# yumcyaWiz/fredholm

Hardware: AMD Instinct MI355X
Metric: Msamples/s at 1920x1080, max_depth=8 (higher is better)
Workload: dtype f32; 1 GPU; configs[2]: 1M random-triangle soup (PCG32 seed 0x853c49e6748fea9b), Hosek sky turbidity 3 albedo 0.3, 1920x1080, max_depth 8, seed 1; triangles=1000000, parallelism=single GPU, gather=none, post=none

## Files before the change

### fredholm_amd/csrc/capi.hip

```cpp
#include <hip/hip_runtime.h>

#include <cmath>
#include <cstdlib>
#include <cstring>

#include "../../include/fredholm/image_io.h"
#include <hip/hip_gl_interop.h>

#include "context.h"
#include "fh_bsdf.h"
#include "fh_local_exposure.h"
#include "fh_meter.h"
#include "fh_trace.h"

#include "gen/tables.inc"

namespace fh {

static thread_local std::string g_create_error;

int fail(fh_ctx* ctx, int code, const std::string& msg)
{
  g_create_error = msg;
  if (ctx) ctx->err = msg;
// ... 154 lines not shown
    int v = 0;
    if (hipDeviceGetAttribute(&v, hipDeviceAttributeMaxSharedMemoryPerMultiprocessor, device) == hipSuccess && v >= 64 * 1024) t.lds_per_cu = (uint32_t)v;
    if (hipDeviceGetAttribute(&v, hipDeviceAttributeSharedMemPerBlockOptin, device) == hipSuccess && v >= 64 * 1024) t.lds_per_block = (uint32_t)v;
    if (t.lds_per_block > t.lds_per_cu) t.lds_per_block = t.lds_per_cu;
    auto env_uint = [](const char* name, int lo, int hi, uint32_t& dst) { if (const char* e = getenv(name)) { const int v = atoi(e); if (v >= lo && v <= hi) dst = (uint32_t)v; } };
    auto env_off = [](const char* name, bool& dst) { if (const char* e = getenv(name)) dst = e[0] != '0'; };
    env_uint("FH_COOP_T", 1, 64, t.coop_flush);
    t.coop_flush_fixed = getenv("FH_COOP_T") != nullptr;
    env_off("FH_COOP", t.coop);
    env_off("FH_STREAM", t.stream);
    t.stream_forced = t.stream && getenv("FH_STREAM") != nullptr;
    env_uint("FH_STREAM_REFILL", 1, 64, t.stream_refill);
    env_uint("FH_STREAM_MIN_RAYS", 0, 65535, t.stream_min_rays);
    env_off("FH_SORT_SMALL", t.sort_small);
    env_off("FH_OVERLAP", t.overlap_secondary);
    env_off("FH_MERGE", t.merge_trace);
    env_uint("FH_SKY_BLOCKS", 0, 64, t.sky_blocks_per_cu);
    env_uint("FH_SKY_FILLER_GRID", 0, 65535, t.sky_filler_grid);
    if (const char* e = getenv("FH_POISON")) t.poison_pools = e[0] == '1';
    env_off("FH_SKY_SPLIT", t.sky_split);
    env_uint("FH_SKY_SPLIT_MIN_LOG2", 0, 40, t.sky_split_min_log2);
    env_uint("FH_STACK_LDS", 1, 99, t.stack_lds_entries);
    env_uint("FH_SHADE_WGS", 2, 3, t.shade_wgs);
    env_uint("FH_STREAM_CHUNK", 16, 65535, t.stream_chunk);
    t.stream_chunk_fixed = getenv("FH_STREAM_CHUNK") != nullptr;
    if (t.stream_chunk_fixed) t.stream_chunk_closest = t.stream_chunk;
    env_uint("FH_STREAM_CHUNK_CLOSEST", 16, 65535, t.stream_chunk_closest);
    env_uint("FH_TAIL_DEPTH", 0, 64, t.tail_depth);
    env_uint("FH_TAIL_PATHS", 64, 1 << 30, t.tail_paths);
    env_off("FH_SORT", t.sort_queues);
    env_uint("FH_SORT_ONEPASS", 0, 2, t.sort_onepass);
    env_uint("FH_BOTTOM_UP", 0, 2, t.bottom_up);
    env_uint("FH_SKY_DEFER", 0, 1, t.sky_defer);
    t.debug_tail = getenv("FH_DEBUG_TAIL") != nullptr;
    if (const char* e = getenv("FH_FORCE_ALPHA")) t.force_alpha = e[0] == '1';
  }
  {
    int least = 0, greatest = 0;
    const char* e = getenv("FH_SKY_PRIO");
    const bool low = !(e && e[0] == '0') && hipDeviceGetStreamPriorityRange(&least, &greatest) == hipSuccess;
    if (ctx->sky_stream.create(hipStreamNonBlocking, low ? least : 0) != hipSuccess) return bail("stream creation failed");
  }
  if (ctx->ev_sky.create(hipEventDisableTiming) != hipSuccess || ctx->ev_sky_cursor.create(hipEventDisableTiming) != hipSuccess) return bail("event creation failed");
  if (ctx->d_split_counters.alloc(4) != hipSuccess) return bail("device allocation failed");
  (void)hipMemsetAsync(ctx->d_split_counters, 0, 16, ctx->stream);
  if (ctx->ev_render_begin.create() != hipSuccess || ctx->ev_render_end.create() != hipSuccess) return bail("event creation failed");
  if (hipStreamSynchronize(ctx->stream) != hipSuccess) return bail("hipStreamSynchronize failed");
  *out = ctx;
  return FH_OK;
}

int fh_ctx_destroy(fh_ctx* ctx)
{
  FH_GROUP(ctx, group_destroy(ctx));
  if (!ctx) return FH_E_INVALID;
  (void)hipSetDevice(ctx->device);
  (void)drain_passes(ctx, true);
  delete ctx;
  return FH_OK;
}

const char* fh_last_error(fh_ctx* ctx) { return ctx ? ctx->err.c_str() : g_create_error.c_str(); }

int fh_set_flags(fh_ctx* ctx, uint32_t flags)
{
  FH_GROUP_EACH(ctx, kGroupCallPlain, fh_set_flags(m_, flags));
  CTX_CHECK(ctx);
  ctx->flags = flags;
  return FH_OK;
}
int fh_get_flags(fh_ctx* ctx, uint32_t* flags)
{
  FH_GROUP_LEAD(ctx);
  CTX_CHECK(ctx);
  if (!flags) return fail(ctx, FH_E_INVALID, "fh_get_flags: null argument");
  *flags = ctx->flags;
  return FH_OK;
}
// ... 783 lines not shown
```

### fredholm_amd/csrc/context.h

```cpp
#pragma once
#include <hip/hip_runtime.h>

#include <functional>
#include <string>
#include <vector>

#include "../../include/fredholm_hip.h"
#include "fh_device.h"
#include "fh_envmap.h"
#include "fh_lights.h"
#include "fh_memory.h"
#include "temporal_host.h"

struct fh_group;

namespace fh { constexpr int kPassSlots = 3; }

struct fh_ctx {
  fh_group* group = nullptr;
  fh_ctx* owner = nullptr;
  uint32_t member_index = 0;
  int device = 0;
  fh::Stream stream;
  fh::Stream aux_stream[fh::kPassSlots - 1];
// ... 49 lines not shown

  fh::DeviceBuffer<float4> d_bvh2_nodes;
  fh::DeviceBuffer<float4> d_bvh2_tris;
  uint32_t bvh2_n_nodes = 0, bvh2_n_tris = 0;
  fh::DeviceBuffer<uint4> d_bvh8_nodes;
  fh::DeviceBuffer<float4> d_bvh8_tris;
  uint32_t bvh8_n_nodes = 0, bvh8_n_tris = 0;
  fh::DeviceBuffer<uint32_t> d_bvh8_parent;
  fh::DeviceBuffer<uint32_t> d_face_node;
  fh::DeviceBuffer<float4> d_bvh8_box;
  std::vector<uint32_t> bvh8_level_start;
  bool refit_ok = false;
  double bvh8_area_built = 0.0;
  uint32_t n_refits = 0;
  uint32_t bvh8_depth = 0;
  uint32_t occupancy_key = 0xffffffffu, occupancy_blocks = 0, occupancy_blocks_secondary = 0;
  uint32_t info_blocks[2] = {0, 0}, info_entries[2] = {0, 0};
  uint32_t lds_configured_bytes = 0;
  uint32_t stream_lds_entries = 0, stream_lds_entries_secondary = 0;
  fh::DeviceBuffer<uint2> d_stack_spill;
  uint32_t lds_static_max = 0;
  bool use_bvh8 = false;
  int builder_choice = 0;
  double bvh_build_ms = 0.0;
  float scene_lo[3] = {0, 0, 0}, scene_hi[3] = {0, 0, 0};

  uint32_t width = 0, height = 0;
  fh::DeviceBuffer<uint32_t> d_sample_count;
  fh::DeviceBuffer<uint32_t> d_sample_issued;
  uint32_t shard_rank = 0, shard_world = 1, tile_w = 32, tile_h = 32;
  fh::DeviceBuffer<uint32_t> d_owned;
  fh::DeviceBuffer<uint32_t> d_owned_xy;
  uint32_t n_owned = 0;
  fh::DeviceBuffer<uint32_t> d_split[4];
  uint32_t n_wave_px = 0, n_sky_px = 0;
  fh::DeviceBuffer<uint32_t> d_split_counters;
  bool split_valid = false;
  float split_key[32] = {};
  fh::Event ev_sky;
  fh::Event ev_sky_cursor;
  struct ShardList { uint32_t rank, world, width, height, tile_w, tile_h; fh::DeviceBuffer<uint32_t> d_owned; uint32_t n_owned; };
  struct FrameMap { uint32_t world = 0, width = 0, height = 0, tile_w = 0, tile_h = 0; fh::DeviceBuffer<uint32_t> d_all; std::vector<uint32_t> start; };
  FrameMap frame_map;
  std::vector<ShardList> shard_lists;
  bool adaptive = false;
  fh_adaptive_params adapt{};
  fh::DeviceBuffer<float2> d_moments;
  bool accumulated = false;
  uint32_t adapt_total = 0;
  fh::DeviceBuffer<uint32_t> d_active[4];
  fh::DeviceBuffer<uint32_t> d_active_blocks;
  fh::PinnedBuffer<uint32_t> h_active_count;
  uint32_t adapt_block = 1, adapt_growth = 1;
  fh::DeviceBuffer<uint32_t> d_block_marks;
  uint32_t mark_seq = 0;
  fh::DeviceBuffer<unsigned long long> d_sky_taken;
  bool sky_taken_pending = false;
  fh::DeviceBuffer<uint8_t> d_sky_adaptive;

  bool has_dir = false;
  float dir_le[3] = {0, 0, 0}, dir_dir[3] = {0, 1, 0}, dir_angle = 0;
  float sky_intensity = 1.0f;
  float sun_dir[3] = {0.0f, 1.0f, 0.0f};
  bool has_hosek = false;
  fh::HosekSky hosek{};
  fh::DeviceBuffer<fh::HosekSky> d_hosek;
  int env_sampling = 0;
  float env_cosine_fraction = FH_ENV_COSINE_FRACTION_DEFAULT;
// ... 52 lines not shown
  std::vector<fh::Event> ev_bounce;
  fh::DeviceBuffer<uint32_t> d_quirk_seen;
  fh::DeviceBuffer<float4> d_quirk_aov;

  struct Tunables {
    uint32_t n_cus = 256;
    uint32_t lds_per_cu = 160u * 1024u, lds_per_block = 160u * 1024u;
    uint32_t coop_flush = 48;
    bool coop_flush_fixed = false;
    bool coop = true;
    bool stream = true;
    bool stream_forced = false;
    uint32_t stream_refill = 24;
    uint32_t stream_min_rays = 64;
    bool overlap_secondary = true;
    bool sky_split = true;
    uint32_t sky_split_min_log2 = 27;
    uint32_t sky_blocks_per_cu = 1;
    uint32_t sky_filler_grid = 0;
    bool poison_pools = false;
    bool merge_trace = true;
    uint32_t shade_wgs = 0;
    uint32_t stack_lds_entries = 0;
    bool sort_small = false;
    uint32_t stream_chunk = 64;
    bool stream_chunk_fixed = false;
    uint32_t stream_chunk_closest = 128;
    uint32_t tail_depth = 0;
    uint32_t tail_paths = 0;
    uint32_t bottom_up = 2;
    bool sort_queues = true;
    uint32_t sort_onepass = 2;
    uint32_t sky_defer = 2;
    bool debug_tail = false;
    bool force_alpha = false;
  } tun;

  fh::DeviceBuffer<float> d_bloom_weights;
  float bloom_sigma_cached = -1.0f, bloom_wsum = 0.0f;

  int auto_exposure = 0;
  fh_auto_exposure_params ae_params = {0.18f, 0.0f, -16.0f, 16.0f, 0.10f, 0.90f, 3.0f, 1.0f, 1.0f / 30.0f, -16.0f, 16.0f, 0u};
  fh::DeviceBuffer<uint8_t> d_meter;
  fh::DeviceBuffer<uint32_t> d_meter_slabs;

  int local_exposure = 0;
  fh_local_exposure_params lx_params = {0.5f, 0.5f, 0.18f, 4.0f, 1.0f, 4u};
  fh::DeviceBuffer<float> d_lx_log;
  fh::DeviceBuffer<float> d_lx_q[2];
  uint32_t lx_w4 = 0, lx_h4 = 0, lx_passes_run = 0;

  fh::DeviceBuffer<float4> d_denoise_tmp[2];
  fh::DeviceBuffer<float4> d_guided_cv[2];
  fh::DeviceBuffer<float> d_guided_var[2];
  struct TemporalHistory {
    fh::DeviceBuffer<float4> d_cv[2], d_ph[2], d_n[2];
    fh::DeviceBuffer<float2> d_mu[2];
    uint32_t w = 0, h = 0, frames = 0;
    int cur = 0;
    fh_camera camera{};
    float w2c[12] = {};
    float inv_tan = 0.0f;
    std::vector<float> o2w, w2o;
    size_t capacity() const { return d_n[1].size(); }
    size_t moment_capacity() const { return d_mu[1].size(); }
    void restart() { frames = 0; }
// ... 137 lines not shown
```

### fredholm_amd/csrc/render.hip

```cpp
#include <hip/hip_runtime.h>

#include <cmath>
#include <cstdio>
#include <cstdlib>
#include <cstring>
#include <type_traits>

#include "context.h"
#include "fh_bsdf.h"
#include "fh_envmap.h"
#include "fh_tonemap.h"
#include "fh_trace.h"
#include "render_plan_host.h"

namespace fh {

namespace {

constexpr int kBlock = 256;
constexpr uint32_t kLutReflFloats = 16 * 16 * 2, kLutSheenFloats = 16 * 16;
constexpr uint32_t kMatLds = 32;
#ifndef FH_SECONDARY_BLOCKS_HEAVY
#define FH_SECONDARY_BLOCKS_HEAVY 5
#endif
#ifndef FH_STREAM_BLOCKS
#define FH_STREAM_BLOCKS 7
#endif
#ifndef FH_STREAM_BLOCKS_ALPHA
#define FH_STREAM_BLOCKS_ALPHA FH_STREAM_BLOCKS
#endif
#ifndef FH_STREAM_BLOCKS_CLOSEST
#define FH_STREAM_BLOCKS_CLOSEST FH_STREAM_BLOCKS
#endif
#ifndef FH_STREAM_BLOCKS_FILLER
#define FH_STREAM_BLOCKS_FILLER 6
#endif
#ifndef FH_SHADE_BLOCKS
#define FH_SHADE_BLOCKS 2
#endif

template <int N>
struct SobolRows {
// ... 100 lines not shown
        pool.rad[p] = mk4(r, 0.0f);
        pool.flags[p] = 2u;
      }
    }
    const unsigned long long m = __ballot(enter);
    if ((threadIdx.x & 63u) == 0u) scratch[4 * c + (threadIdx.x >> 6)] = (uint32_t)__popcll(m);
    packed |= ((enter ? 0x80u : 0u) | (uint32_t)__popcll(m & ((1ull << (threadIdx.x & 63u)) - 1ull))) << (8 * c);
   }
   __syncthreads();
   if (threadIdx.x == 0u) {
     uint32_t total = 0;
     for (uint32_t c = 0; c < 4u * kGenChunks; ++c) { const uint32_t v = scratch[c]; scratch[c] = total; total += v; }
     scratch[4 * kGenChunks] = total ? atomicAdd(&pool.counters[CNT_RAD], total) : 0u;
   }
   __syncthreads();
   ++iter;
#pragma unroll
   for (int c = 0; c < kGenChunks; ++c)
     if ((packed >> (8 * c)) & 0x80u)
       pool.q_rad[0][scratch[4 * kGenChunks] + scratch[4 * c + (threadIdx.x >> 6)] + ((packed >> (8 * c)) & 63u)] = k * n_owned + base + (uint32_t)c * blockDim.x + threadIdx.x;
  }
}

__global__ void __launch_bounds__(kBlock) k_bump_issued(uint32_t* issued, const uint32_t* owned, uint32_t n_owned, uint32_t n_batch)
{
  const uint32_t i = blockIdx.x * blockDim.x + threadIdx.x;
  if (i < n_owned) issued[owned[i]] += n_batch;
}

struct SplitDev {
  f3 centre;
  float radius;
  float far;
  uint32_t* wave_px; uint32_t* wave_xy; uint32_t* sky_px; uint32_t* sky_xy;
  uint32_t* counters;
};
__global__ void __launch_bounds__(kBlock) k_split_pixels(FrameDev fr, SplitDev sp, const uint32_t* owned, const uint32_t* owned_xy, uint32_t n_owned)
{
  __shared__ uint32_t s_reserve[2][10];
  uint32_t iter = 0;
  for (uint32_t base = blockIdx.x * blockDim.x; base < n_owned; base += gridDim.x * blockDim.x) {
    const uint32_t i = base + threadIdx.x;
    bool sky = false, wave = false;
    uint32_t px = 0, xy = 0;
    if (i < n_owned) {
      px = owned[i]; xy = owned_xy[i];
      const float x = (float)(xy & 0xffffu) + 0.5f, y = (float)(xy >> 16) + 0.5f;
      const float uvx = -(2.0f * x - (float)fr.width) / (float)fr.height, uvy = (2.0f * y - (float)fr.height) / (float)fr.height;
      const float f = fr.cam_inv_tan, k = 1.0f - fr.cam_a_plus_b / f;
      const f3 a0 = mk3(0.0f, 0.0f, f), b0 = mk3(k * uvx, k * uvy, 2.0f * f - fr.cam_a_plus_b);
      const f3 ab = b0 - a0;
      const float L = length(ab);
      const float m = fabsf(fr.cam_lens_radius) + 1.41421357f * fabsf(k) / (float)fr.height * 1.001f;
      const f3 w = sp.centre - a0;
      const float tau = dot(w, ab) / L;
      const float d0 = sqrt_cr(fmaxf(dot(w, w) - tau * tau, 0.0f));
      const float q = 1.0f - (m / L) * (m / L);
      const float nearest = d0 * sqrt_cr(fmaxf(q, 0.0f)) - fabsf(fr.cam_lens_radius) - m * fabsf(tau) / L;
      sky = L > 0.0f && q > 0.0f && nearest > sp.radius * 1.001f + 1e-3f * (length(w) + 1.0f);
      if (!sky && L > m * 1.01f) {
        const float d = (fabsf(fr.cam_lens_radius) + m * (sp.far + fabsf(fr.cam_lens_radius)) / (L - m)) * 1.001f + 1e-3f * (sp.far + 1.0f);
        const f3 o = xform_point(fr.cam_xf, a0), dir = xform_dir(fr.cam_xf, (1.0f / L) * ab);
        float tn = -3.0e38f, tf = 3.0e38f;
        bool miss = false;
        const float oo[3] = {o.x, o.y, o.z}, dd[3] = {dir.x, dir.y, dir.z}, lo[3] = {fr.scene_lo.x - d, fr.scene_lo.y - d, fr.scene_lo.z - d}, hi[3] = {fr.scene_hi.x + d, fr.scene_hi.y + d, fr.scene_hi.z + d};
#pragma unroll
        for (int a = 0; a < 3; ++a) {
          if (fabsf(dd[a]) < 1e-12f) miss = miss || oo[a] < lo[a] || oo[a] > hi[a];
          else {
            const float t0 = (lo[a] - oo[a]) / dd[a], t1 = (hi[a] - oo[a]) / dd[a];
            tn = fmaxf(tn, fminf(t0, t1)); tf = fminf(tf, fmaxf(t0, t1));
          }
        }
        miss = miss || tn - 1e-3f * (fabsf(tn) + sp.far) > tf + 1e-3f * (fabsf(tf) + sp.far);
        sky = miss && dd[0] == dd[0] && dd[1] == dd[1] && dd[2] == dd[2] && d == d;
      }
      wave = !sky;
    }
    uint32_t* const counters2[2] = {sp.counters, sp.counters + 1};
    const bool act[2] = {wave, sky};
    uint32_t pos[2];
    block_queue_reserve<2>(counters2, act, pos, s_reserve[iter & 1u]);
    ++iter;
    if (wave) { sp.wave_px[pos[0]] = px; sp.wave_xy[pos[0]] = xy; }
    if (sky) { sp.sky_px[pos[1]] = px; sp.sky_xy[pos[1]] = xy; }
  }
}

struct AdaptiveDev {
  float2* moments;
  const uint32_t* count;
  float threshold, floor;
  uint32_t min_samples, step;
  uint32_t growth, b0;
  uint32_t* marks;
  uint32_t tag, block_shift, blocks_x, width;
};

FH_D bool adaptive_boundary(const AdaptiveDev& ad, uint32_t n)
{
  if (ad.growth == 1u) return n >= ad.min_samples && n % ad.step == 0u;
  if (ad.b0 == 0u || n < ad.b0 || n % ad.b0 != 0u) return false;
  const uint32_t q = n / ad.b0;
  return (q & (q - 1u)) == 0u;
}

FH_D bool adaptive_converged(const AdaptiveDev& ad, uint32_t n, float m1, float m2)
{
  if (!adaptive_boundary(ad, n)) return false;
  float d = m2 - m1 * m1;
  if (d < 0.0f) d = 0.0f;
  const float var = d * ((float)n / (float)(n - 1u));
  const float e2 = var / (float)n;
  const float ref = m1 > ad.floor ? m1 : ad.floor;
  const float t = ad.threshold * ref;
  return ad.threshold > 0.0f && e2 <= t * t;
}

// ... 80 lines not shown
                              __float_as_uint(tcx) | __float_as_uint(tcy);
    if (any_bits != 0u) {
      uint32_t n_aov = n_spp - taken;
#pragma unroll 1
      for (uint32_t k = 0; k < taken; ++k) {
        const float coef = div_r_nofix<0, 0, 0, 32>(1.0f, n_aov + 1.0f);
        const float fn = (float)n_aov;
        position = coef * (fn * position + mk3(0.0f));
        normal = coef * (fn * normal + mk3(0.0f));
        depth = coef * (fn * depth + 0.0f);
        tcx = coef * (fn * tcx + 0.0f);
        tcy = coef * (fn * tcy + 0.0f);
        albedo = coef * (fn * albedo + mk3(0.0f));
        n_aov++;
      }
    }
    layers.position[image_idx] = mk4(position, 1.0f);
    layers.normal[image_idx] = mk4(normal, 1.0f);
    layers.depth[image_idx] = depth;
    layers.texcoord[image_idx] = make_float4(tcx, tcy, 0.0f, 1.0f);
    layers.albedo[image_idx] = mk4(albedo, 1.0f);
    }
  }
  if constexpr (ADAPTIVE) {
    __shared__ unsigned long long s_taken;
    if (threadIdx.x == 0u) s_taken = 0ull;
    __syncthreads();
    if (n_taken) atomicAdd(&s_taken, n_taken);
    __syncthreads();
    if (threadIdx.x == 0u && s_taken) atomicAdd(violations_or_adaptive->taken, s_taken);
  }
}

FH_D bool adaptive_unconverged(const AdaptiveDev& ad, uint32_t image_idx)
{
  const float2 m = ad.moments[image_idx];
  return !adaptive_converged(ad, ad.count[image_idx], m.x, m.y);
}

FH_D bool adaptive_active(const AdaptiveDev& ad, uint32_t image_idx)
{
  if (ad.marks) {
    const uint32_t y = image_idx / ad.width, x = image_idx - y * ad.width;
    return ad.marks[(y >> ad.block_shift) * ad.blocks_x + (x >> ad.block_shift)] == ad.tag;
  }
  return adaptive_unconverged(ad, image_idx);
}

__global__ void __launch_bounds__(kBlock) k_adaptive_mark(AdaptiveDev ad, const uint32_t* owned_px, const uint32_t* owned_xy, uint32_t n_owned)
{
  const uint32_t i = blockIdx.x * kBlock + threadIdx.x;
  uint32_t key = 0xffffffffu;
  if (i < n_owned && adaptive_unconverged(ad, owned_px[i])) {
    const uint32_t xy = owned_xy[i];
    key = ((xy >> 16) >> ad.block_shift) * ad.blocks_x + ((xy & 0xffffu) >> ad.block_shift);
  }
  const uint32_t below = __shfl_up(key, 1);
  if (key != 0xffffffffu && ((threadIdx.x & 63u) == 0u || below != key)) ad.marks[key] = ad.tag;
}

__global__ void __launch_bounds__(kBlock) k_adaptive_count(AdaptiveDev ad, const uint32_t* base_px, uint32_t n_base, uint32_t* blocks)
{
  __shared__ uint32_t s_w[kBlock / 64];
  const uint32_t i = blockIdx.x * kBlock + threadIdx.x;
  const bool act = i < n_base && adaptive_active(ad, base_px[i]);
  const unsigned long long m = __ballot(act);
// ... 1567 lines not shown
      }); });
  set((const void*)k_tail<L_DIFF>);
  set((const void*)k_tail<L_METAL | L_SPEC | L_DIFF>);
  set((const void*)k_tail<L_COAT | L_METAL | L_SPEC | L_DIFF>);
  set((const void*)k_tail<L_ALL>);
  set((const void*)k_tail_env<L_DIFF>);
  set((const void*)k_tail_env<L_METAL | L_SPEC | L_DIFF>);
  set((const void*)k_tail_env<L_COAT | L_METAL | L_SPEC | L_DIFF>);
  set((const void*)k_tail_env<L_ALL>);
  for (int e = 0; e < 2; ++e)
    with_bool(e != 0, [&](auto E) {
      set((const void*)k_tail_lt<L_DIFF, decltype(E)::value>);
      set((const void*)k_tail_lt<L_METAL | L_SPEC | L_DIFF, decltype(E)::value>);
      set((const void*)k_tail_lt<L_COAT | L_METAL | L_SPEC | L_DIFF, decltype(E)::value>);
      set((const void*)k_tail_lt<L_ALL, decltype(E)::value>);
    });
  for (int a = 0; a < 2; ++a)
    with_bool(a != 0, [&](auto A) {
      set((const void*)MergedStreamFn<const float*>(k_trace_merged_stream<true, decltype(A)::value>));
      for (int c = 0; c < 2; ++c)
        with_bool(c != 0, [&](auto C) {
          set((const void*)SecondaryStreamFn<const float*>(k_trace_secondary_stream<decltype(C)::value, true, decltype(A)::value>));
          set((const void*)SecondaryCoopFn<const float*>(k_trace_secondary_coop<decltype(C)::value, true, decltype(A)::value>));
          set((const void*)SecondaryStaticFn<const float*>(k_trace_secondary_static<decltype(C)::value, true, true, decltype(A)::value>));
          set((const void*)SecondaryStaticFn<const float*>(k_trace_secondary_static<decltype(C)::value, false, true, decltype(A)::value>));
        });
    });
  if (err != hipSuccess) return fail(ctx, FH_E_HIP, std::string("hipFuncSetAttribute(MaxDynamicSharedMemorySize): ") + hipGetErrorString(err));
  ctx->lds_configured_bytes = stack_bytes;
  ctx->lds_static_max = max_static;
  return FH_OK;
}

static int split_pixels(fh_ctx* ctx, const fh_camera* cam, const FrameDev& fr)
{
  float key[32] = {};
  for (int i = 0; i < 12; ++i) key[i] = cam->transform[i];
  key[12] = cam->fov; key[13] = cam->F; key[14] = cam->focus;
  for (int i = 0; i < 3; ++i) { key[15 + i] = ctx->scene_lo[i]; key[18 + i] = ctx->scene_hi[i]; }
  key[21] = (float)ctx->width; key[22] = (float)ctx->height; key[23] = (float)ctx->n_owned; key[24] = (float)ctx->shard_rank; key[25] = (float)ctx->shard_world;
  key[26] = (float)ctx->tile_w; key[27] = (float)ctx->tile_h;
  if (ctx->split_valid && std::memcmp(key, ctx->split_key, sizeof key) == 0) return FH_OK;
  ctx->split_valid = false;
  const float* t = cam->transform;
  float dev = 0.0f;
  for (int a = 0; a < 3; ++a)
    for (int b = 0; b < 3; ++b) {
      const float d = t[a] * t[b] + t[4 + a] * t[4 + b] + t[8 + a] * t[8 + b];
      dev = fmaxf(dev, fabsf(d - (a == b ? 1.0f : 0.0f)));
    }
  std::memcpy(ctx->split_key, key, sizeof key);
  ctx->n_wave_px = ctx->n_owned; ctx->n_sky_px = 0;
  if (!(dev < 1e-4f)) { ctx->split_valid = true; return FH_OK; }
  if (ctx->d_split[3].size() < ctx->n_owned) {
    FH_HIP(hipDeviceSynchronize());
    for (int k = 0; k < 4; ++k) ctx->d_split[k].reset();
    for (int k = 0; k < 4; ++k) FH_HIP(ctx->d_split[k].alloc(ctx->n_owned));
  }
  FH_HIP(drain_passes(ctx, true));
  SplitDev sp{};
  const float c[3] = {0.5f * (ctx->scene_lo[0] + ctx->scene_hi[0]), 0.5f * (ctx->scene_lo[1] + ctx->scene_hi[1]), 0.5f * (ctx->scene_lo[2] + ctx->scene_hi[2])};
  const float w[3] = {c[0] - t[3], c[1] - t[7], c[2] - t[11]};
  sp.centre = mk3(t[0] * w[0] + t[4] * w[1] + t[8] * w[2], t[1] * w[0] + t[5] * w[1] + t[9] * w[2], t[2] * w[0] + t[6] * w[1] + t[10] * w[2]);
  const float e[3] = {ctx->scene_hi[0] - ctx->scene_lo[0], ctx->scene_hi[1] - ctx->scene_lo[1], ctx->scene_hi[2] - ctx->scene_lo[2]};
  sp.radius = 0.5f * sqrtf(e[0] * e[0] + e[1] * e[1] + e[2] * e[2]);
  {
    const float f = fr.cam_inv_tan, a0w[3] = {t[2] * f + t[3], t[6] * f + t[7], t[10] * f + t[11]};
    float far2 = 0.0f;
    for (int k = 0; k < 8; ++k) {
      float d2 = 0.0f;
      for (int a = 0; a < 3; ++a) { const float c = ((k >> a) & 1) ? ctx->scene_hi[a] : ctx->scene_lo[a]; d2 += (c - a0w[a]) * (c - a0w[a]); }
      far2 = fmaxf(far2, d2);
    }
    sp.far = sqrtf(far2) * 1.001f;
  }
  sp.wave_px = ctx->d_split[0]; sp.wave_xy = ctx->d_split[1]; sp.sky_px = ctx->d_split[2]; sp.sky_xy = ctx->d_split[3];
  sp.counters = ctx->d_split_counters;
  FH_HIP(hipMemsetAsync(ctx->d_split_counters, 0, 8, ctx->stream));
  hipLaunchKernelGGL(k_split_pixels, dim3(grid_for(ctx->n_owned)), dim3(kBlock), 0, ctx->stream, fr, sp, ctx->d_owned, ctx->d_owned_xy, ctx->n_owned);
  uint32_t n[2] = {0, 0};
  FH_HIP(hipMemcpyAsync(n, ctx->d_split_counters, 8, hipMemcpyDeviceToHost, ctx->stream));
  FH_HIP(hipStreamSynchronize(ctx->stream));
  if (n[0] + n[1] != ctx->n_owned) return fail(ctx, FH_E_HIP, "k_split_pixels lost pixels");
  ctx->n_wave_px = n[0]; ctx->n_sky_px = n[1];
  ctx->split_valid = true;
  if (getenv("FH_DEBUG_BVH")) fprintf(stderr, "[split] %u of %u owned pixels cannot see the scene (bounding sphere radius %.4f at camera-space (%.3f, %.3f, %.3f))\n", n[1], ctx->n_owned, sp.radius, sp.centre.x, sp.centre.y, sp.centre.z);
  return FH_OK;
}

static unsigned long long adaptive_b0(const fh_ctx* ctx)
{
  const unsigned long long step = ctx->adapt.step ? ctx->adapt.step : 1u;
  return (ctx->adapt.min_samples + step - 1ull) / step * step;
}

static AdaptiveDev adaptive_dev(const fh_ctx* ctx)
{
  const unsigned long long b0 = adaptive_b0(ctx);
  uint32_t shift = 0;
  while ((1u << shift) < ctx->adapt_block) ++shift;
  return AdaptiveDev{ctx->d_moments, ctx->d_sample_count, ctx->adapt.threshold, ctx->adapt.floor, ctx->adapt.min_samples, ctx->adapt.step,
                     ctx->adapt_growth, b0 <= 0xffffffffull ? (uint32_t)b0 : 0u,
                     ctx->adapt_block > 1u ? ctx->d_block_marks : nullptr, ctx->mark_seq, shift, (ctx->width + ctx->adapt_block - 1u) >> shift, ctx->width};
}

uint32_t adaptive_to_boundary(const fh_ctx* ctx)
{
  const unsigned long long t = ctx->adapt_total, b0 = adaptive_b0(ctx);
  unsigned long long next = b0;
  if (t >= b0) {
    if (ctx->adapt_growth == 1u) next = t - t % ctx->adapt.step + ctx->adapt.step;
    else while (next <= t) next *= 2ull;
  }
  return next - t > 0xffffffffull ? 0xffffffffu : (uint32_t)(next - t);
}

int adaptive_upload(fh_ctx* ctx)
{
  FH_HIP(ctx->d_sky_adaptive.ensure(sizeof(SkyAdaptive)));
// ... 90 lines not shown
  fr.cam_inv_tan = 1.0f / tanf(0.5f * cam->fov);
  fr.cam_F = cam->F; fr.cam_focus = cam->focus;
  lens_values(fr.cam_inv_tan, cam->focus, cam->F, &fr.cam_a_plus_b, &fr.cam_lens_radius);
  fr.bg = mk3(bg[0], bg[1], bg[2]);
  fr.sky_intensity = ctx->sky_intensity;
  fr.sun_dir = mk3(ctx->sun_dir[0], ctx->sun_dir[1], ctx->sun_dir[2]);
  fr.hosek = ctx->d_hosek;
  fr.dir_le = mk3(ctx->dir_le[0], ctx->dir_le[1], ctx->dir_le[2]);
  fr.dir_dir = mk3(ctx->dir_dir[0], ctx->dir_dir[1], ctx->dir_dir[2]);
  fr.dir_disk_radius = 1e9f * tanf(0.5f * ctx->dir_angle * kPi / 180.0f);
  fr.scene_lo = mk3(ctx->scene_lo[0], ctx->scene_lo[1], ctx->scene_lo[2]);
  fr.scene_hi = mk3(ctx->scene_hi[0], ctx->scene_hi[1], ctx->scene_hi[2]);
  {
    const float cells = (float)(1u << kCellBits);
    const float ex = ctx->scene_hi[0] - ctx->scene_lo[0], ey = ctx->scene_hi[1] - ctx->scene_lo[1], ez = ctx->scene_hi[2] - ctx->scene_lo[2];
    fr.cell_scale = mk3(ex > 0.0f ? cells / ex : 0.0f, ey > 0.0f ? cells / ey : 0.0f, ez > 0.0f ? cells / ez : 0.0f);
  }
  fr.sobol = ctx->d_sobol;
  fr.sobol_bytes = ctx->d_sobol_bytes;
  fr.lut.reflection = ctx->d_lut_refl;
  fr.lut.sheen = ctx->d_lut_sheen;
  return fr;
}

LayersDev layers_dev(const fh_ctx* ctx, const fh_render_layers* layers)
{
  LayersDev L{};
  L.beauty = (float4*)layers->beauty; L.position = (float4*)layers->position; L.depth = layers->depth;
  L.normal = (float4*)layers->normal; L.texcoord = (float4*)layers->texcoord; L.albedo = (float4*)layers->albedo;
  L.sample_count = ctx->d_sample_count;
  return L;
}

struct PixelLists { const uint32_t* px; const uint32_t* xy; uint32_t n_px, n_sky; };

int choose_pixels(fh_ctx* ctx, const fh_camera* cam, const FrameDev& fr, uint32_t n_samples, bool quirk, PixelLists& out)
{
  out = PixelLists{ctx->d_owned, ctx->d_owned_xy, ctx->n_owned, 0u};
  if (!(ctx->tun.sky_split && !quirk && (unsigned long long)n_samples * ctx->n_owned >= (1ull << ctx->tun.sky_split_min_log2))) return FH_OK;
  const int rc = split_pixels(ctx, cam, fr);
  if (rc) return rc;
  if (ctx->split_valid && ctx->n_sky_px >= ctx->n_owned / 8u)
    out = PixelLists{ctx->d_split[0], ctx->d_split[1], ctx->n_wave_px, ctx->n_sky_px};
  return FH_OK;
}

int quirk_begin(fh_ctx* ctx)
{
  const size_t px = (size_t)ctx->width * ctx->height;
  if (ctx->d_quirk_aov.size() != px * 4) {
    ctx->d_quirk_seen.reset(); ctx->d_quirk_aov.reset();
    FH_HIP(ctx->d_quirk_seen.alloc(px));
    FH_HIP(ctx->d_quirk_aov.alloc(px * 4));
  }
  FH_HIP(hipMemsetAsync(ctx->d_quirk_seen, 0, px * sizeof(uint32_t), ctx->stream));
  FH_HIP(hipMemsetAsync(ctx->d_quirk_aov, 0, px * 4 * sizeof(float4), ctx->stream));
  return FH_OK;
}

struct SkyLaunches {
  fh_ctx* ctx;
  const FrameDev& fr;
  const LayersDev& L;
  bool adaptive;
  hipStream_t st;
  uint32_t* cursor;
  uint32_t filler_wgs, full_wgs;
  struct Drain { const uint32_t* px; const uint32_t* xy; uint32_t n, n_samples; bool pending; } drain{nullptr, nullptr, 0u, 0u, false};

  SkyLaunches(fh_ctx* c, const FrameDev& f, const LayersDev& l, bool a)
      : ctx(c), fr(f), L(l), adaptive(a), st(((c->flags & FH_FLAG_SERIAL_PASSES) != 0 || c->n_slots == 1) ? c->stream : c->sky_stream), cursor(c->d_split_counters + 3),
        filler_wgs(st == c->stream ? 0u : (c->tun.sky_filler_grid ? c->tun.sky_filler_grid : c->tun.n_cus * c->tun.sky_blocks_per_cu)),
        full_wgs(c->tun.n_cus * (uint32_t)kSkyWaves)
  {
  }
  void launch(hipStream_t s, uint32_t wgs, const uint32_t* px, const uint32_t* xy, uint32_t n, uint32_t ns)
// ... 417 lines not shown
  const bool quirk = (ctx->flags & FH_FLAG_REFERENCE_FIRSTHIT) != 0 && n_samples > 1;
  if (adaptive && quirk)
    return fail(ctx, FH_E_INVALID, "fh_render: FH_FLAG_REFERENCE_FIRSTHIT with n_samples > 1 does not combine with adaptive sampling (its first-hit state is per launch)");
  ctx->accumulated = true;
  cap_pool_target(ctx);

  const bool count = (ctx->flags & FH_FLAG_COUNT_TRAVERSAL) != 0;
  unsigned long long* const tc = ctx->d_trace_counters;
  const bool clocks = (ctx->flags & FH_FLAG_TIME_KERNELS) != 0;
  Call c{ctx, frame_dev(ctx, cam, bg, seed, max_depth), layers_dev(ctx, layers), SceneDev{},
         TraceCounters{tc, tc + 1, tc + 2, tc + 6, tc + 7, tc + 10, clocks ? tc + 27 : nullptr}, TraceCounters{tc + 3, tc + 4, tc + 5, tc + 8, tc + 9, tc + 18, clocks ? tc + 29 : nullptr},
         max_depth, adaptive, quirk, count, StreamPlan{}, env_table_dev(ctx), ctx->env_sampling != 0, light_table_dev(ctx), ctx->light_sampling != 0 && ctx->n_lights > 0};
  if (c.lt_on) { const int rc = light_table_ensure(ctx); if (rc) return rc; c.lt = light_table_dev(ctx); }
  if (c.env_on) { const int rc = env_table_ensure(ctx); if (rc) return rc; }
  PixelLists base;
  { const int rc = choose_pixels(ctx, cam, c.fr, n_samples, quirk, base); if (rc) return rc; }
  const uint32_t target = ctx->pool_target > ctx->n_owned ? ctx->pool_target : ctx->n_owned;
  c.sc = scene_dev(ctx);
  if (quirk) { const int rc = quirk_begin(ctx); if (rc) return rc; }
  if (!ctx->render_pending) { (void)hipEventRecord(ctx->ev_render_begin, ctx->stream); ctx->render_pending = true; }
  FH_HIP(hipEventRecord(ctx->ev_enter, ctx->stream));
  for (int k = 0; k + 1 < ctx->n_slots; ++k) FH_HIP(hipStreamWaitEvent(ctx->aux_stream[k], ctx->ev_enter, 0));
  SkyLaunches sky(ctx, c.fr, c.L, adaptive);
  if (base.n_sky && sky.st != ctx->stream) FH_HIP(hipStreamWaitEvent(sky.st, ctx->ev_enter, 0));
  if (base.n_sky && !guard_blocks) {
    const int rc = sky.begin(ctx->d_split[2], ctx->d_split[3], base.n_sky, n_samples);
    if (rc) return rc;
    if (adaptive) ctx->sky_taken_pending = true;
    else {
      ctx->stats.paths += (uint64_t)base.n_sky * n_samples;
      ctx->stats.sky_pixel_samples += (uint64_t)base.n_sky * n_samples;
    }
  }
  { const int rc = stream_plan(ctx, c.sc, count, base.n_sky && sky.filler_wgs, c.plan); if (rc) return rc; }
  if (ctx->tun.debug_tail) {
    if (!ctx->d_resolve_dbg) FH_HIP(ctx->d_resolve_dbg.alloc(2));
    FH_HIP(hipMemsetAsync(ctx->d_resolve_dbg, 0, 2 * sizeof(unsigned long long), ctx->stream));
    FH_HIP(hipEventRecord(ctx->ev_enter, ctx->stream));
    for (int k = 0; k + 1 < ctx->n_slots; ++k) FH_HIP(hipStreamWaitEvent(ctx->aux_stream[k], ctx->ev_enter, 0));
  }

  PixelLists act = base;
  act.n_sky = 0;
  bool ran = false, sky_ran = false;
  int last_slot = 0;
  for (uint32_t call_done = 0; call_done < n_samples;) {
    uint32_t n_round = n_samples - call_done;
    if (adaptive) {
      const uint32_t to_boundary = ctx->adapt_growth == 1u ? ctx->adapt.step - ctx->adapt_total % ctx->adapt.step : adaptive_to_boundary(ctx);
      if (n_round > to_boundary) n_round = to_boundary;
      const int rc = select_round(c, sky, base, guard_blocks, ran ? last_slot : 0, n_round, act, sky_ran);
      if (rc) return rc;
    }
    const uint32_t batch = samples_per_pass(target, act.n_px, n_round, (uint32_t)ctx->n_slots, quirk, (ctx->flags & FH_FLAG_SERIAL_PASSES) != 0);
    const uint32_t coop_flush = (!ctx->tun.coop_flush_fixed && batch >= n_round && !c.sc.has_alpha && ctx->tun.coop_flush > 32u) ? 32u : ctx->tun.coop_flush;
    for (uint32_t done = 0; done < n_round && act.n_px; done += batch) {
      ran = true;
      const int rc = submit_pass(c, act, (n_round - done) < batch ? (n_round - done) : batch, batch, n_round, coop_flush, last_slot);
      if (rc) return rc;
    }
    call_done += n_round;
    ctx->adapt_total += n_round;
    if (adaptive && act.n_px == 0 && act.n_sky == 0) { ctx->adapt_total += n_samples - call_done; break; }
  }
  if (last_slot != 0 && ran) FH_HIP(hipStreamWaitEvent(ctx->stream, ctx->slot[last_slot].ev_acc, 0));
  sky.end();
  if (base.n_sky && sky.st != ctx->stream) { FH_HIP(hipEventRecord(ctx->ev_sky, sky.st)); FH_HIP(hipStreamWaitEvent(ctx->stream, ctx->ev_sky, 0)); }
  FH_HIP(hipGetLastError());
  if (ctx->tun.debug_tail) {
    unsigned long long dbg[2] = {0ull, 0ull};
    FH_HIP(hipStreamSynchronize(ctx->stream));
    FH_HIP(hipMemcpy(dbg, ctx->d_resolve_dbg, sizeof(dbg), hipMemcpyDeviceToHost));
    if (dbg[1]) fprintf(stderr, "[sky-resolve] %llu queue entries, %llu escaped sky / light rays: %.4f per entry\n", dbg[1], dbg[0], (double)dbg[0] / (double)dbg[1]);
  }
  return FH_OK;
}

}
```

### fredholm_amd/csrc/render_plan_host.h

```cpp
#pragma once
#include <cmath>
#include <cstdint>

namespace fh {

inline uint32_t pool_target_cap(unsigned long long free_bytes, unsigned long long held, uint32_t pool_share, int n_slots, unsigned long long bytes_per_path, uint32_t target_default,
                                uint32_t n_owned)
{
  const unsigned long long cap = (free_bytes + held) / (4ull * pool_share) / ((unsigned long long)n_slots * bytes_per_path);
  if (cap < target_default) return cap > n_owned ? (uint32_t)cap : n_owned;
  return target_default;
}

inline uint32_t samples_per_pass(uint32_t target, uint32_t n_px, uint32_t n_samples, uint32_t n_slots, bool quirk, bool serial)
{
  uint32_t batch = n_px ? target / n_px : n_samples;
  if (batch > n_samples) batch = n_samples;
  if (batch > 65535u) batch = 65535u;
  if (batch < 1) batch = 1;
  if (batch < n_samples) {
    uint32_t passes = (n_samples + batch - 1u) / batch;
    if (n_slots > 1u && passes > n_slots && passes % n_slots != 0u && (passes / n_slots + 1u) * n_slots <= n_samples) passes = (passes / n_slots + 1u) * n_slots;
    batch = (n_samples + passes - 1u) / passes;
  }
// ... 78 lines not shown
  for (uint32_t d = 0; d < wave_depth; ++d) { c += kNodeRoundCycles * counters[d * stride + node_index] + kTriRoundCycles * counters[d * stride + tri_index]; n += counters[d * stride + sec_index]; }
  *cost += c; *items += n;
}

inline int bottom_up_verdict(const double cost[2], const double items[2])
{
  if (!(items[0] >= 65536.0 && items[1] >= 65536.0)) return 0;
  const double off = cost[0] / items[0], on = cost[1] / items[1];
  return on < 0.95 * off ? 2 : 1;
}

inline void lens_values(float inv_tan, float focus, float F, float* a_plus_b, float* lens_radius)
{
  volatile float f = inv_tan, b = focus;
  volatile float inv_b = 1.0f / b;
  volatile float den = 1.0f + f;
  den = den - inv_b;
  volatile float a = 1.0f / den;
  volatile float apb = a + b;
  volatile float two_f = 2.0f * f;
  volatile float lr = two_f / F;
  *a_plus_b = apb;
  *lens_radius = lr;
}

inline bool sky_defer_verdict(bool emitters, bool hosek, bool ibl, bool env_sampling, bool light_tables, bool stream_secondary, bool merged, bool shade_three, uint32_t forced, bool by_default)
{
  const bool eligible = !emitters && (hosek || ibl) && !env_sampling && !light_tables && stream_secondary && !merged && shade_three;
  if (forced == 0u) return false;
  if (forced == 1u) return eligible;
  return eligible && by_default;
}

}
```

Measured before the change: 8540 Msamples/s.

## Classify below-horizon sky pixels as dark and write zero radiance analytically

Adds a third class to the pixel split: camera rays that miss the scene bounds and point below the Hosek sky horizon (with a conservative margin) are queued separately. A small kernel then accumulates zero radiance and zero AOVs for those pixels instead of running the sky-evaluation path. This removes per-sample sky shading work for pixels whose Hosek radiance is zero, at the cost of an extra queue, a kernel launch and a conservative geometric test that must stay exact.

```diff
diff --git a/fredholm_amd/csrc/capi.hip b/fredholm_amd/csrc/capi.hip
--- a/fredholm_amd/csrc/capi.hip
+++ b/fredholm_amd/csrc/capi.hip
@@ -210,6 +210,7 @@
     env_uint("FH_SORT_ONEPASS", 0, 2, t.sort_onepass);
     env_uint("FH_BOTTOM_UP", 0, 2, t.bottom_up);
     env_uint("FH_SKY_DEFER", 0, 1, t.sky_defer);
+    env_uint("FH_DARK_SKY", 0, 1, t.dark_sky);
     t.debug_tail = getenv("FH_DEBUG_TAIL") != nullptr;
     if (const char* e = getenv("FH_FORCE_ALPHA")) t.force_alpha = e[0] == '1';
   }
@@ -220,8 +221,8 @@
     if (ctx->sky_stream.create(hipStreamNonBlocking, low ? least : 0) != hipSuccess) return bail("stream creation failed");
   }
   if (ctx->ev_sky.create(hipEventDisableTiming) != hipSuccess || ctx->ev_sky_cursor.create(hipEventDisableTiming) != hipSuccess) return bail("event creation failed");
-  if (ctx->d_split_counters.alloc(4) != hipSuccess) return bail("device allocation failed");
-  (void)hipMemsetAsync(ctx->d_split_counters, 0, 16, ctx->stream);
+  if (ctx->d_split_counters.alloc(5) != hipSuccess) return bail("device allocation failed");
+  (void)hipMemsetAsync(ctx->d_split_counters, 0, 20, ctx->stream);
   if (ctx->ev_render_begin.create() != hipSuccess || ctx->ev_render_end.create() != hipSuccess) return bail("event creation failed");
   if (hipStreamSynchronize(ctx->stream) != hipSuccess) return bail("hipStreamSynchronize failed");
   *out = ctx;
diff --git a/fredholm_amd/csrc/context.h b/fredholm_amd/csrc/context.h
--- a/fredholm_amd/csrc/context.h
+++ b/fredholm_amd/csrc/context.h
@@ -105,8 +105,8 @@
   fh::DeviceBuffer<uint32_t> d_owned;
   fh::DeviceBuffer<uint32_t> d_owned_xy;
   uint32_t n_owned = 0;
-  fh::DeviceBuffer<uint32_t> d_split[4];
-  uint32_t n_wave_px = 0, n_sky_px = 0;
+  fh::DeviceBuffer<uint32_t> d_split[6];
+  uint32_t n_wave_px = 0, n_sky_px = 0, n_dark_px = 0;
   fh::DeviceBuffer<uint32_t> d_split_counters;
   bool split_valid = false;
   float split_key[32] = {};
@@ -225,6 +225,7 @@
     bool sort_queues = true;
     uint32_t sort_onepass = 2;
     uint32_t sky_defer = 2;
+    uint32_t dark_sky = 2;
     bool debug_tail = false;
     bool force_alpha = false;
   } tun;
diff --git a/fredholm_amd/csrc/fh_dark_sky.h b/fredholm_amd/csrc/fh_dark_sky.h
--- /dev/null
+++ b/fredholm_amd/csrc/fh_dark_sky.h
@@ -0,0 +1,19 @@
+#pragma once
+#if defined(__HIPCC__)
+#include "fh_vec.h"
+#elif !defined(FH_HD)
+#define FH_HD inline
+#endif
+
+namespace fh {
+
+constexpr float kDarkMargin = 0.0009765625f;
+
+FH_HD bool dark_sky_pixel(float cy, float m, float L)
+{
+  if (!(L > 1.01f * m)) return false;
+  const float spread = 2.0f * m / (L - m) * 1.001f + 1e-3f;
+  return cy + spread < -kDarkMargin;
+}
+
+}
diff --git a/fredholm_amd/csrc/render.hip b/fredholm_amd/csrc/render.hip
--- a/fredholm_amd/csrc/render.hip
+++ b/fredholm_amd/csrc/render.hip
@@ -8,6 +8,7 @@
 
 #include "context.h"
 #include "fh_bsdf.h"
+#include "fh_dark_sky.h"
 #include "fh_envmap.h"
 #include "fh_tonemap.h"
 #include "fh_trace.h"
@@ -174,16 +175,17 @@
   f3 centre;
   float radius;
   float far;
-  uint32_t* wave_px; uint32_t* wave_xy; uint32_t* sky_px; uint32_t* sky_xy;
+  uint32_t dark_on;
+  uint32_t* wave_px; uint32_t* wave_xy; uint32_t* sky_px; uint32_t* sky_xy; uint32_t* dark_px; uint32_t* dark_xy;
   uint32_t* counters;
 };
 __global__ void __launch_bounds__(kBlock) k_split_pixels(FrameDev fr, SplitDev sp, const uint32_t* owned, const uint32_t* owned_xy, uint32_t n_owned)
 {
-  __shared__ uint32_t s_reserve[2][10];
+  __shared__ uint32_t s_reserve[2][15];
   uint32_t iter = 0;
   for (uint32_t base = blockIdx.x * blockDim.x; base < n_owned; base += gridDim.x * blockDim.x) {
     const uint32_t i = base + threadIdx.x;
-    bool sky = false, wave = false;
+    bool sky = false, wave = false, dark = false;
     uint32_t px = 0, xy = 0;
     if (i < n_owned) {
       px = owned[i]; xy = owned_xy[i];
@@ -218,14 +220,20 @@
         sky = miss && dd[0] == dd[0] && dd[1] == dd[1] && dd[2] == dd[2] && d == d;
       }
       wave = !sky;
-    }
-    uint32_t* const counters2[2] = {sp.counters, sp.counters + 1};
-    const bool act[2] = {wave, sky};
-    uint32_t pos[2];
-    block_queue_reserve<2>(counters2, act, pos, s_reserve[iter & 1u]);
+      if (sky && sp.dark_on) {
+        const f3 c = xform_dir(fr.cam_xf, (1.0f / L) * ab);
+        dark = c.x == c.x && c.z == c.z && dark_sky_pixel(c.y, m, L);
+        sky = !dark;
+      }
+    }
+    uint32_t* const counters3[3] = {sp.counters, sp.counters + 1, sp.counters + 4};
+    const bool act[3] = {wave, sky, dark};
+    uint32_t pos[3];
+    block_queue_reserve<3>(counters3, act, pos, s_reserve[iter & 1u]);
     ++iter;
     if (wave) { sp.wave_px[pos[0]] = px; sp.wave_xy[pos[0]] = xy; }
     if (sky) { sp.sky_px[pos[1]] = px; sp.sky_xy[pos[1]] = xy; }
+    if (dark) { sp.dark_px[pos[2]] = px; sp.dark_xy[pos[2]] = xy; }
   }
 }
 
@@ -372,6 +380,55 @@
   }
 }
 
+__global__ void __launch_bounds__(kBlock) k_dark_pixels(LayersDev layers, uint32_t* issued, const uint32_t* dark_px, uint32_t n_dark, uint32_t n_samples)
+{
+  for (uint32_t i = blockIdx.x * blockDim.x + threadIdx.x; i < n_dark; i += gridDim.x * blockDim.x) {
+    const uint32_t image_idx = dark_px[i];
+    const uint32_t first = layers.sample_count[image_idx];
+    f3 beauty = mk3(layers.beauty[image_idx]);
+    if ((__float_as_uint(beauty.x) | __float_as_uint(beauty.y) | __float_as_uint(beauty.z)) != 0u) {
+      uint32_t n_spp = first;
+#pragma unroll 1
+      for (uint32_t k = 0; k < n_samples; ++k) {
+        const float coef = div_r_nofix<0, 0, 0, 32>(1.0f, n_spp + 1.0f);
+        const float fn = (float)n_spp;
+        beauty = coef * (fn * beauty + mk3(0.0f));
+        n_spp++;
+      }
+    }
+    f3 position = mk3(layers.position[image_idx]), normal = mk3(layers.normal[image_idx]), albedo = mk3(layers.albedo[image_idx]);
+    float depth = layers.depth[image_idx];
+    const float4 tc4 = layers.texcoord[image_idx];
+    float tcx = tc4.x, tcy = tc4.y;
+    const uint32_t any_bits = __float_as_uint(position.x) | __float_as_uint(position.y) | __float_as_uint(position.z) | __float_as_uint(normal.x) | __float_as_uint(normal.y) |
+                              __float_as_uint(normal.z) | __float_as_uint(albedo.x) | __float_as_uint(albedo.y) | __float_as_uint(albedo.z) | __float_as_uint(depth) |
+                              __float_as_uint(tcx) | __float_as_uint(tcy);
+    if (any_bits != 0u) {
+      uint32_t n_aov = first;
+#pragma unroll 1
+      for (uint32_t k = 0; k < n_samples; ++k) {
+        const float coef = div_r_nofix<0, 0, 0, 32>(1.0f, n_aov + 1.0f);
+        const float fn = (float)n_aov;
+        position = coef * (fn * position + mk3(0.0f));
+        normal = coef * (fn * normal + mk3(0.0f));
+        depth = coef * (fn * depth + 0.0f);
+        tcx = coef * (fn * tcx + 0.0f);
+        tcy = coef * (fn * tcy + 0.0f);
+        albedo = coef * (fn * albedo + mk3(0.0f));
+        n_aov++;
+      }
+    }
+    issued[image_idx] += n_samples;
+    layers.sample_count[image_idx] = first + n_samples;
+    layers.beauty[image_idx] = mk4(beauty, 1.0f);
+    layers.position[image_idx] = mk4(position, 1.0f);
+    layers.normal[image_idx] = mk4(normal, 1.0f);
+    layers.depth[image_idx] = depth;
+    layers.texcoord[image_idx] = make_float4(tcx, tcy, 0.0f, 1.0f);
+    layers.albedo[image_idx] = mk4(albedo, 1.0f);
+  }
+}
+
 FH_D bool adaptive_unconverged(const AdaptiveDev& ad, uint32_t image_idx)
 {
   const float2 m = ad.moments[image_idx];
@@ -2005,7 +2062,7 @@
   return FH_OK;
 }
 
-static int split_pixels(fh_ctx* ctx, const fh_camera* cam, const FrameDev& fr)
+static int split_pixels(fh_ctx* ctx, const fh_camera* cam, const FrameDev& fr, bool dark)
 {
   float key[32] = {};
   for (int i = 0; i < 12; ++i) key[i] = cam->transform[i];
@@ -2013,6 +2070,7 @@
   for (int i = 0; i < 3; ++i) { key[15 + i] = ctx->scene_lo[i]; key[18 + i] = ctx->scene_hi[i]; }
   key[21] = (float)ctx->width; key[22] = (float)ctx->height; key[23] = (float)ctx->n_owned; key[24] = (float)ctx->shard_rank; key[25] = (float)ctx->shard_world;
   key[26] = (float)ctx->tile_w; key[27] = (float)ctx->tile_h;
+  key[28] = dark ? 1.0f : 0.0f;
   if (ctx->split_valid && std::memcmp(key, ctx->split_key, sizeof key) == 0) return FH_OK;
   ctx->split_valid = false;
   const float* t = cam->transform;
@@ -2023,12 +2081,12 @@
       dev = fmaxf(dev, fabsf(d - (a == b ? 1.0f : 0.0f)));
     }
   std::memcpy(ctx->split_key, key, sizeof key);
-  ctx->n_wave_px = ctx->n_owned; ctx->n_sky_px = 0;
+  ctx->n_wave_px = ctx->n_owned; ctx->n_sky_px = 0; ctx->n_dark_px = 0;
   if (!(dev < 1e-4f)) { ctx->split_valid = true; return FH_OK; }
-  if (ctx->d_split[3].size() < ctx->n_owned) {
+  if (ctx->d_split[5].size() < ctx->n_owned) {
     FH_HIP(hipDeviceSynchronize());
-    for (int k = 0; k < 4; ++k) ctx->d_split[k].reset();
-    for (int k = 0; k < 4; ++k) FH_HIP(ctx->d_split[k].alloc(ctx->n_owned));
+    for (int k = 0; k < 6; ++k) ctx->d_split[k].reset();
+    for (int k = 0; k < 6; ++k) FH_HIP(ctx->d_split[k].alloc(ctx->n_owned));
   }
   FH_HIP(drain_passes(ctx, true));
   SplitDev sp{};
@@ -2047,17 +2105,19 @@
     }
     sp.far = sqrtf(far2) * 1.001f;
   }
-  sp.wave_px = ctx->d_split[0]; sp.wave_xy = ctx->d_split[1]; sp.sky_px = ctx->d_split[2]; sp.sky_xy = ctx->d_split[3];
+  sp.wave_px = ctx->d_split[0]; sp.wave_xy = ctx->d_split[1]; sp.sky_px = ctx->d_split[2]; sp.sky_xy = ctx->d_split[3]; sp.dark_px = ctx->d_split[4]; sp.dark_xy = ctx->d_split[5];
+  sp.dark_on = dark ? 1u : 0u;
   sp.counters = ctx->d_split_counters;
   FH_HIP(hipMemsetAsync(ctx->d_split_counters, 0, 8, ctx->stream));
+  FH_HIP(hipMemsetAsync(ctx->d_split_counters + 4, 0, 4, ctx->stream));
   hipLaunchKernelGGL(k_split_pixels, dim3(grid_for(ctx->n_owned)), dim3(kBlock), 0, ctx->stream, fr, sp, ctx->d_owned, ctx->d_owned_xy, ctx->n_owned);
-  uint32_t n[2] = {0, 0};
-  FH_HIP(hipMemcpyAsync(n, ctx->d_split_counters, 8, hipMemcpyDeviceToHost, ctx->stream));
+  uint32_t n[5] = {0, 0, 0, 0, 0};
+  FH_HIP(hipMemcpyAsync(n, ctx->d_split_counters, sizeof n, hipMemcpyDeviceToHost, ctx->stream));
   FH_HIP(hipStreamSynchronize(ctx->stream));
-  if (n[0] + n[1] != ctx->n_owned) return fail(ctx, FH_E_HIP, "k_split_pixels lost pixels");
-  ctx->n_wave_px = n[0]; ctx->n_sky_px = n[1];
+  if ((unsigned long long)n[0] + n[1] + n[4] != ctx->n_owned || (!dark && n[4])) return fail(ctx, FH_E_HIP, "k_split_pixels lost pixels");
+  ctx->n_wave_px = n[0]; ctx->n_sky_px = n[1]; ctx->n_dark_px = n[4];
   ctx->split_valid = true;
-  if (getenv("FH_DEBUG_BVH")) fprintf(stderr, "[split] %u of %u owned pixels cannot see the scene (bounding sphere radius %.4f at camera-space (%.3f, %.3f, %.3f))\n", n[1], ctx->n_owned, sp.radius, sp.centre.x, sp.centre.y, sp.centre.z);
+  if (getenv("FH_DEBUG_BVH")) fprintf(stderr, "[split] %u of %u owned pixels cannot see the scene, %u of them dark (bounding sphere radius %.4f at camera-space (%.3f, %.3f, %.3f))\n", n[1] + n[4], ctx->n_owned, n[4], sp.radius, sp.centre.x, sp.centre.y, sp.centre.z);
   return FH_OK;
 }
 
@@ -2214,16 +2274,18 @@
   return L;
 }
 
-struct PixelLists { const uint32_t* px; const uint32_t* xy; uint32_t n_px, n_sky; };
+struct PixelLists { const uint32_t* px; const uint32_t* xy; uint32_t n_px, n_sky, n_dark; };
 
 int choose_pixels(fh_ctx* ctx, const fh_camera* cam, const FrameDev& fr, uint32_t n_samples, bool quirk, PixelLists& out)
 {
-  out = PixelLists{ctx->d_owned, ctx->d_owned_xy, ctx->n_owned, 0u};
-  if (!(ctx->tun.sky_split && !quirk && (unsigned long long)n_samples * ctx->n_owned >= (1ull << ctx->tun.sky_split_min_log2))) return FH_OK;
-  const int rc = split_pixels(ctx, cam, fr);
+  out = PixelLists{ctx->d_owned, ctx->d_owned_xy, ctx->n_owned, 0u, 0u};
+  const bool splits = ctx->tun.sky_split && !quirk && (unsigned long long)n_samples * ctx->n_owned >= (1ull << ctx->tun.sky_split_min_log2);
+  if (!splits) return FH_OK;
+  const bool dark = dark_sky_verdict(splits, fr.has_hosek != 0, fr.has_ibl != 0, ctx->adaptive, (ctx->flags & FH_FLAG_REFERENCE_FIRSTHIT) != 0, ctx->tun.dark_sky);
+  const int rc = split_pixels(ctx, cam, fr, dark);
   if (rc) return rc;
-  if (ctx->split_valid && ctx->n_sky_px >= ctx->n_owned / 8u)
-    out = PixelLists{ctx->d_split[0], ctx->d_split[1], ctx->n_wave_px, ctx->n_sky_px};
+  if (ctx->split_valid && ctx->n_sky_px + ctx->n_dark_px >= ctx->n_owned / 8u)
+    out = PixelLists{ctx->d_split[0], ctx->d_split[1], ctx->n_wave_px, ctx->n_sky_px, ctx->n_dark_px};
   return FH_OK;
 }
 
@@ -2707,6 +2769,12 @@
       ctx->stats.sky_pixel_samples += (uint64_t)base.n_sky * n_samples;
     }
   }
+  if (base.n_dark) {
+    Span sp(ctx, ctx->stream, 4);
+    hipLaunchKernelGGL(k_dark_pixels, dim3(grid_for(base.n_dark)), dim3(kBlock), 0, ctx->stream, c.L, ctx->d_sample_issued, (const uint32_t*)ctx->d_split[4].get(), base.n_dark, n_samples);
+    ctx->stats.paths += (uint64_t)base.n_dark * n_samples;
+    ctx->stats.sky_pixel_samples += (uint64_t)base.n_dark * n_samples;
+  }
   { const int rc = stream_plan(ctx, c.sc, count, base.n_sky && sky.filler_wgs, c.plan); if (rc) return rc; }
   if (ctx->tun.debug_tail) {
     if (!ctx->d_resolve_dbg) FH_HIP(ctx->d_resolve_dbg.alloc(2));
@@ -2746,6 +2814,7 @@
     unsigned long long dbg[2] = {0ull, 0ull};
     FH_HIP(hipStreamSynchronize(ctx->stream));
     FH_HIP(hipMemcpy(dbg, ctx->d_resolve_dbg, sizeof(dbg), hipMemcpyDeviceToHost));
+    if (base.n_sky || base.n_dark) fprintf(stderr, "[dark-sky] %u of %u sky pixels are dark\n", base.n_dark, base.n_sky + base.n_dark);
     if (dbg[1]) fprintf(stderr, "[sky-resolve] %llu queue entries, %llu escaped sky / light rays: %.4f per entry\n", dbg[1], dbg[0], (double)dbg[0] / (double)dbg[1]);
   }
   return FH_OK;
diff --git a/fredholm_amd/csrc/render_plan_host.h b/fredholm_amd/csrc/render_plan_host.h
--- a/fredholm_amd/csrc/render_plan_host.h
+++ b/fredholm_amd/csrc/render_plan_host.h
@@ -134,4 +134,10 @@
   return eligible && by_default;
 }
 
+inline bool dark_sky_verdict(bool splits_sky, bool hosek, bool ibl, bool adaptive, bool reference_firsthit, uint32_t forced)
+{
+  const bool eligible = splits_sky && hosek && !ibl && !adaptive && !reference_firsthit;
+  return forced != 0u && eligible;
 }
+
+}
```

Measured after the change: 8876 Msamples/s (median of 6 runs). 3.9% higher.
